# aidanmrli/rwm-pt-pytorch

Measured on AMD Instinct MI355X. Metric: chain-MH-steps/sec, higher is better.
Workload: dtype f32; 1 GPU; BASELINE configs[2]: PT-RWM HIP, RoughCarpet dim=30 modes[-15,0,15], Normal proposal 2.38^2/dim, 32 geometric temps 1->0.01, swap_every=10, 65536 ladders per GPU; dim=30, temps=32, ladders_per_gpu=65536, mh_steps_per_launch=2000, swap_every=10, swap_mode=exchange, swap_order=sequential, rng=Philox4x32-10 in-kernel, world_size=1

## Files before the change

### rwm-pt-pytorch_amd/csrc/kernel.h

```cpp
#pragma once
#include "philox.h"
#include "proposals.h"
#include "targets.h"

namespace ptrwm {

#ifndef PTRWM_BLOCK_THREADS
#define PTRWM_BLOCK_THREADS 256
#endif
constexpr int kBlockThreads = PTRWM_BLOCK_THREADS;
constexpr int kWavesPerBlock = kBlockThreads / 64;
constexpr int kLdsExtraPerThread = 8;
constexpr int kLdsStreamStatPerThread = 5;
constexpr int kStreamSlabs = 2;
constexpr int lds_floats_per_thread(int dp, bool stream) {
  return (stream ? kStreamSlabs * (dp + kLdsStreamStatPerThread) : dp) + kLdsExtraPerThread;
}
constexpr unsigned step_kernel_lds_bytes(int threads, int dp, bool stream = false) {
  return (unsigned)(threads * lds_floats_per_thread(dp, stream)) * 4u;
}
constexpr unsigned kWideVoteBytes = 16u;

struct FullArgs {
  const float *__restrict__ ext_prop;
  const float *__restrict__ ext_u;
  const float *__restrict__ ext_swap_u;
  float *__restrict__ trace;
  float *__restrict__ trace_logp;
  unsigned char *__restrict__ accept_flags;
  long long trace_chains, trace_row0;
  int trace_temps, n_raw_ext;
  int trace_every;
  int steps_to_trace;
  double *__restrict__ mom_sum;
  double *__restrict__ mom_sum_sq;
  double *__restrict__ mom_sum_logp;
  long long *__restrict__ mom_count;
  long long mom_steps;
  int mom_temps, mom_every;
  int steps_to_mom;
};

typedef const __attribute__((address_space(4))) FullArgs *kargs_full_ptr;

struct KArgs {
  float *__restrict__ state;
  float *__restrict__ logp;
  const float *__restrict__ beta;
  const float *__restrict__ temp_scale;
  long long *__restrict__ n_accept;
  double *__restrict__ sq_jump;
  long long *__restrict__ swap_accept;
  long long *__restrict__ last_swap_ordinal;
  long long n_chains, chain_offset, step0;
  long long first_swap_event;
  int n_steps;
  int burn_left;
  int n_temps, dim, swap_every, swap_mode, swap_order, chains_per_wave;
  int steps_to_swap;
  unsigned k0, k1;
  TParams tp;
  PParams pp;
  FullArgs full;
};

__device__ __forceinline__ float swap_log_prob(float bj, float bk, float lj, float lk) {
  return sub_rn(sub_rn(add_rn(mul_rn(bj, lk), mul_rn(bk, lj)), mul_rn(bj, lj)), mul_rn(bk, lk));
}

__device__ __forceinline__ bool swap_accept_test(float u, float log_prob) {
  const float threshold = (log_prob >= 0.0f) ? 1.0f : hw_exp(log_prob);
  return u < threshold;
}

__device__ __forceinline__ bool mh_accept(float beta_t, float lp_new, float lp, float u_acc) {
  const float ratio = mul_rn(beta_t, sub_rn(lp_new, lp));
  return (ratio > 0.0f) || (u_acc < hw_exp(ratio));
}

__device__ __forceinline__ bool swap_pair_plain(int T, int t, float db, float lp, float us) {
  const bool last = t >= T - 1;
  const float u = last ? 0.5f : us;
  const float d = last ? 1.0f : db;
  const float inside = mul_rn(u, sub_rn(1.0f, u));
  return add_rn(__builtin_fminf(inside, d), mul_rn(lp, 0.0f)) > 0.0f;
}
__device__ __forceinline__ bool ladder_votes_plain(bool mine, int first_lane, int lanes_per_ladder) {
  const unsigned long long against = __builtin_amdgcn_ballot_w64(!mine);
  const unsigned long long ladder = (lanes_per_ladder >= 64 ? ~0ull : ((1ull << lanes_per_ladder) - 1ull)) << first_lane;
  return (against & ladder) == 0ull;
}

template <class Sync>
__device__ __forceinline__ void swap_decide(int T, int t, int base, int slot, int swap_mode, int swap_order, int par,
                                            const float *__restrict__ beta, float beta_t, float us, const float *s_l,
                                            float *s_u, int *landed, float &my_l, int &src, bool &pair_acc, Sync sync,
                                            bool plain) {
  if (swap_order == PTRWM_ORDER_SEQUENTIAL) {
    if (swap_mode == PTRWM_SWAP_EXCHANGE) {
      const bool has_k = t < T - 1;
      const float db = has_k ? sub_rn(beta_t, beta[t + 1]) : 1.0f;
      float car_l = s_l[base];
      int car_i = base;
      if (plain) {
        const float lk = s_l[has_k ? slot + 1 : slot];
        s_u[slot] = fmaf(-hw_ln(us), __builtin_amdgcn_rcpf(db), lk);
        sync();
#pragma unroll 2
        for (int j = 0; j < T - 1; ++j) {
          const int ik = base + j + 1;
          const float lkj = s_l[ik];
          const bool ok = car_l < s_u[base + j];
          landed[base + j] = ok ? ik : car_i;
          car_l = ok ? car_l : lkj;
          car_i = ok ? car_i : ik;
        }
      } else {
#pragma unroll 2
        for (int j = 0; j < T - 1; ++j) {
          const float lk = s_l[base + j + 1];
          const float u = s_u[base + j];
          const float bj = beta[j], bk = beta[j + 1];
          const bool ok = swap_accept_test(u, swap_log_prob(bj, bk, car_l, lk));
          const int ik = base + j + 1;
          landed[base + j] = ok ? ik : car_i;
          car_l = ok ? car_l : lk;
          car_i = ok ? car_i : ik;
        }
      }
      landed[base + T - 1] = car_i;
      src = landed[base + t];
      my_l = s_l[src];
      pair_acc = (t < T - 1) && (src == base + t + 1);
    } else {
      if (t < T - 1) {
        const float lk = s_l[slot + 1];
        const bool ok = swap_accept_test(us, swap_log_prob(beta_t, beta[t + 1], my_l, lk));
        if (ok) {
          my_l = lk;
          src = slot + 1;
        }
        pair_acc = ok;
      }
    }
  } else {
    const bool lower = ((t & 1) == par);
    const int partner_t = lower ? t + 1 : t - 1;
    const bool valid = partner_t >= 0 && partner_t < T;
    if (valid) {
      const int partner = base + partner_t;
      const float l_other = s_l[partner];
      const float u_low = lower ? us : s_u[partner];
      const int tj = lower ? t : partner_t;
      const float lj = lower ? my_l : l_other;
      const float lk = lower ? l_other : my_l;
      const bool ok = swap_accept_test(u_low, swap_log_prob(beta[tj], beta[tj + 1], lj, lk));
      if (ok && (lower || swap_mode == PTRWM_SWAP_EXCHANGE)) {
        my_l = l_other;
        src = partner;
      }
      pair_acc = ok && lower;
    }
  }
}

__device__ __forceinline__ int stage_head(const float *g) { return (int)((reinterpret_cast<uintptr_t>(g) >> 2) & 3u); }

template <bool LOAD>
__device__ __forceinline__ void stage_copy(float *__restrict__ lds, float *__restrict__ g, int total, int tid, int nthr) {
  typedef float vec4 __attribute__((ext_vector_type(4)));
  const int head = stage_head(g);
  vec4 *__restrict__ gv = reinterpret_cast<vec4 *>(g - head);
  vec4 *__restrict__ lv = reinterpret_cast<vec4 *>(lds);
  const int v_lo = head ? 1 : 0;
  const int v_hi = (head + total) >> 2;
  constexpr int kDepth = 4;
  int v0 = v_lo + tid;
  for (; v0 + (kDepth - 1) * nthr < v_hi; v0 += kDepth * nthr) {
    vec4 t[kDepth];
#pragma unroll
    for (int k = 0; k < kDepth; ++k) t[k] = LOAD ? gv[v0 + k * nthr] : lv[v0 + k * nthr];
#pragma unroll
    for (int k = 0; k < kDepth; ++k) (LOAD ? lv : gv)[v0 + k * nthr] = t[k];
  }
  if (v0 < v_hi) {
    vec4 t[kDepth - 1];
#pragma unroll
    for (int k = 0; k < kDepth - 1; ++k) {
      const int v = v0 + k * nthr;
      if (v < v_hi) t[k] = LOAD ? gv[v] : lv[v];
    }
#pragma unroll
    for (int k = 0; k < kDepth - 1; ++k) {
      const int v = v0 + k * nthr;
      if (v < v_hi) (LOAD ? lv : gv)[v] = t[k];
    }
  }
  const int e_lo = (4 * v_lo - head < total) ? 4 * v_lo - head : total;
  const int e_hi = (4 * v_hi - head > e_lo) ? 4 * v_hi - head : e_lo;
  if (tid < 6) {
    const int i = tid < 3 ? tid : e_hi + (tid - 3);
    const bool mine = tid < 3 ? (i < e_lo) : (i < total);
    if (mine) {
      if (LOAD) lds[head + i] = g[i];
      else g[i] = lds[head + i];
    }
  }
}

__device__ __forceinline__ int wave_in_block() { return __builtin_amdgcn_readfirstlane((int)(threadIdx.x >> 6)); }
__device__ __forceinline__ int thread_index_now(int wave) {
  unsigned all = ~0u;
  PTRWM_VALUE_BARRIER("+s"(all));
  return wave * 64 + (int)__builtin_amdgcn_mbcnt_hi(all, __builtin_amdgcn_mbcnt_lo(all, 0u));
}

__device__ __forceinline__ void count_add(long long *p, long long v) {
  (void)__hip_atomic_fetch_add(p, v, __ATOMIC_RELAXED, __HIP_MEMORY_SCOPE_AGENT);
}

constexpr unsigned moments_region_doubles(int temps, int dim) { return (unsigned)(temps * (2 * dim + 1)); }

__device__ __forceinline__ void moments_zero(double *reg, int n, int tid, int nthr) {
  for (int i = tid; i < n; i += nthr) reg[i] = 0.0;
}
__device__ __forceinline__ void moments_add(double *p, double v) {
  (void)__hip_atomic_fetch_add(p, v, __ATOMIC_RELAXED, __HIP_MEMORY_SCOPE_WORKGROUP);
}
__device__ __forceinline__ void moments_flush(const double *reg, kargs_full_ptr f, int dim, long long live_ladders, int tid,
                                              int nthr) {
  const int temps = f->mom_temps;
  const int td = temps * dim;
  double *const sum = f->mom_sum, *const sum_sq = f->mom_sum_sq, *const sum_logp = f->mom_sum_logp;
  const int n = 2 * td + (sum_logp != nullptr ? temps : 0);
  for (int i = tid; i < n; i += nthr) {
    const double v = reg[i];
    if (v != 0.0) unsafeAtomicAdd(i < td ? sum + i : (i < 2 * td ? sum_sq + (i - td) : sum_logp + (i - 2 * td)), v);
  }
  long long *const count = f->mom_count;
  const long long add = live_ladders * f->mom_steps;
  if (count != nullptr)
    for (int i = tid; i < temps; i += nthr) count_add(&count[i], add);
}

template <int DP>
__device__ __forceinline__ double *thread_moments_region(float *s_dyn, bool wide, int gthreads, int wave, int stride) {
  float *const base = s_dyn + (wide ? gthreads * (DP + kLdsExtraPerThread) + (int)(kWideVoteBytes / 4u)
                                    : kBlockThreads * (DP + kLdsExtraPerThread));
  return reinterpret_cast<double *>(base) + (wide ? 0 : wave * stride);
}

template <bool EXACT>
__device__ __forceinline__ int fresh_dim(int d0) {
  if constexpr (!EXACT) PTRWM_VALUE_BARRIER("+s"(d0));
  return d0;
}

typedef const __attribute__((address_space(4))) KArgs *kargs_ptr;
__device__ __forceinline__ kargs_ptr late_args() {
  uintptr_t p = (uintptr_t)__builtin_amdgcn_kernarg_segment_ptr();
  PTRWM_VALUE_BARRIER("+s"(p));
  return (kargs_ptr)p;
}

#ifndef PTRWM_J2_FENCE_MASK
#define PTRWM_J2_FENCE_MASK 7
#endif
#ifndef PTRWM_WAVES_SMALL
#define PTRWM_WAVES_SMALL 4
#endif
#ifndef PTRWM_WAVES_40
#define PTRWM_WAVES_40 3
#endif
#ifndef PTRWM_WAVES_MID
#define PTRWM_WAVES_MID 2
#endif
constexpr int min_waves_per_simd(int dp) {
  return dp <= 30 ? PTRWM_WAVES_SMALL : (dp <= 44 ? PTRWM_WAVES_40 : (dp <= 64 ? PTRWM_WAVES_MID : 1));
}
constexpr bool step_loop_at_register_cap(int dp, bool stream) { return !stream && min_waves_per_simd(dp) >= 4 && dp > 24; }

constexpr int stream_waves_per_simd(int dp) {
  return dp <= 10 ? 4 : (dp <= 20 ? 2 : (dp <= 30 ? 2 : 1));
}

constexpr int stream_register_waves(int dp) { return stream_waves_per_simd(dp) < 2 ? 2 : stream_waves_per_simd(dp); }

template <class Target, class Proposal, int DP, bool EXACT, bool FULL, bool STREAM = false>
__global__ void __launch_bounds__(kBlockThreads, STREAM ? stream_register_waves(DP) : min_waves_per_simd(DP)) ptrwm_step_kernel(const KArgs a) {
  static_assert(!(STREAM && FULL), "the streaming form is a production kernel: no fixture / trace arguments");
  const int T = a.n_temps;
  const int D0 = EXACT ? DP : a.dim;
  const int cpw = a.chains_per_wave;
  const bool wide = !STREAM && T > 64;
  const int wave = wave_in_block();
  const int tid = wide ? (int)threadIdx.x : (int)(threadIdx.x & 63);
  long long group = STREAM ? (long long)blockIdx.x * kWavesPerBlock + wave
                           : (wide ? (long long)blockIdx.x : (long long)blockIdx.x * kWavesPerBlock + (threadIdx.x >> 6));
  [[maybe_unused]] const long long n_groups = STREAM ? a.n_chains / cpw : 0;
  [[maybe_unused]] const long long group_stride = STREAM ? (long long)gridDim.x * kWavesPerBlock : 0;
  if (STREAM ? (group >= n_groups) : (group * cpw >= a.n_chains)) return;
  extern __shared__ __attribute__((aligned(16))) float s_dyn[];
  typedef float pf_vec4 __attribute__((ext_vector_type(4)));
  constexpr int NV = STREAM ? (DP + 3) / 4 : 1;
  constexpr int kWaveFloats = 64 * lds_floats_per_thread(DP, STREAM);
  constexpr int kExtra0 = 64 * kStreamSlabs * DP;
  constexpr int kZone0 = kExtra0 + 64 * kLdsExtraPerThread, kZoneFloats = 64 * kLdsStreamStatPerThread;
  [[maybe_unused]] int cur = 0;
  typedef const __attribute__((address_space(1))) void *dma_src;
  typedef __attribute__((address_space(3))) void *dma_dst;
  [[maybe_unused]] auto prefetch = [&](long long g, int slab) {
    const int tid = thread_index_now(wave) & 63;
    const kargs_ptr ap = late_args();
    const int n_vec = (cpw * T * D0) >> 2;
    const int n_live = cpw * T;
    float *const wbase = s_dyn + wave * kWaveFloats;
    const long long r0 = g * n_live;
    float *const zone = wbase + kZone0 + slab * kZoneFloats;
    __builtin_amdgcn_global_load_lds((dma_src)(ap->logp + r0 + (tid < n_live ? tid : 0)), (dma_dst)(uintptr_t)zone, 4, 0, 0);
    if (ap->sq_jump != nullptr && 2 * tid < n_live)
      __builtin_amdgcn_global_load_lds((dma_src)(ap->sq_jump + r0 + 2 * tid), (dma_dst)(uintptr_t)(zone + 64), 16, 0, 0);
    if (ap->n_accept != nullptr && 2 * tid < n_live)
      __builtin_amdgcn_global_load_lds((dma_src)(ap->n_accept + r0 + 2 * tid), (dma_dst)(uintptr_t)(zone + 192), 16, 0, 0);
    const pf_vec4 *__restrict__ gv = reinterpret_cast<const pf_vec4 *>(ap->state + g * cpw * T * (long long)D0);
    float *const dst = wbase + slab * (64 * DP);
#pragma unroll
    for (int k = 0; k < NV; ++k) {
      const int v = tid + 64 * k;
      if (v < n_vec) __builtin_amdgcn_global_load_lds((dma_src)(gv + v), (dma_dst)(uintptr_t)(dst + 256 * k), 16, 0, 0);
    }
  };
  [[maybe_unused]] float beta_t_s = 0.0f, tscale_s = 0.0f;
  [[maybe_unused]] float db_s = 1.0f;
  [[maybe_unused]] pf_vec4 pend_o[NV];
  [[maybe_unused]] float pend_lp = 0.0f;
  [[maybe_unused]] unsigned pend_n_swap = 0u;
  [[maybe_unused]] long long pend_acc = 0;
  [[maybe_unused]] bool pend_acc_on = false;
  [[maybe_unused]] double pend_sq = 0.0;
  [[maybe_unused]] long long pend_ord = 0, pend_group = 0;
  [[maybe_unused]] bool pend_sq_on = false, pend_ord_on = false, have_pending = false;
  [[maybe_unused]] auto flush_pending = [&]() {
    const kargs_ptr ap = late_args();
    const int tid = thread_index_now(wave) & 63;
    const int n_live = cpw * T;
    const int n_vec = (n_live * D0) >> 2;
    pf_vec4 *__restrict__ gv = reinterpret_cast<pf_vec4 *>(ap->state + pend_group * n_live * (long long)D0);
#pragma unroll
    for (int k = 0; k < NV; ++k) {
      const int v = tid + 64 * k;
      if (v < n_vec) gv[v] = pend_o[k];
    }
    if (tid < n_live) {
      const long long r = pend_group * n_live + tid;
      ap->logp[r] = pend_lp;
      if (pend_acc_on) ap->n_accept[r] = pend_acc;
      if (pend_sq_on) ap->sq_jump[r] = pend_sq;
      if (ap->swap_accept != nullptr && pend_n_swap != 0u) count_add(&ap->swap_accept[r], (long long)pend_n_swap);
      if (pend_ord_on) (void)__hip_atomic_fetch_max(&ap->last_swap_ordinal[r], pend_ord, __ATOMIC_RELAXED, __HIP_MEMORY_SCOPE_AGENT);
    }
  };
  if constexpr (STREAM) {
    const int cw_s = tid / T;
    const int t_s = cw_s < cpw ? tid - cw_s * T : 0;
    beta_t_s = a.beta[t_s];
    tscale_s = a.temp_scale[t_s];
    db_s = sub_rn(beta_t_s, a.beta[t_s < T - 1 ? t_s + 1 : t_s]);
    prefetch(group, 0);
  }
  do {
  const long long chain0 = group * cpw;
  const int cw_raw = tid / T;
  const int t_raw = tid - cw_raw * T;
  const bool live = (cw_raw < cpw) && (chain0 + cw_raw < a.n_chains);
  const int cw = live ? cw_raw : 0;
  const int t = live ? t_raw : 0;
  const long long chain = chain0 + cw;
  const long long rep = chain0 * T + (live ? tid : 0);

  float *const s_stage = STREAM ? s_dyn + wave * kWaveFloats + cur * (64 * DP)
                                : s_dyn + (wide ? 0 : (int)(threadIdx.x >> 6) * (64 * (DP + kLdsExtraPerThread)));
  [[maybe_unused]] float *const s_extra = s_dyn + wave * kWaveFloats + kExtra0;
  auto sync_group = [&]() {
    if (wide) {
      __syncthreads();
    } else {
      __builtin_amdgcn_fence(__ATOMIC_ACQ_REL, "wavefront");
      __builtin_amdgcn_wave_barrier();
    }
  };

  float x[DP], y[DP];
  {
    const long long live_chains = (a.n_chains - chain0 < cpw) ? (a.n_chains - chain0) : cpw;
    const int stage_total = (int)live_chains * T * D0;
    float *__restrict__ gs = a.state + chain0 * T * (long long)D0;
    const int nthr = wide ? ((T + 63) & ~63) : 64;
    int row_head = 0;
    if constexpr (!STREAM) {
      stage_copy<true>(s_stage, gs, stage_total, tid, nthr);
      row_head = stage_head(gs);
      if (wide) reinterpret_cast<int *>(s_dyn)[nthr * (DP + kLdsExtraPerThread)] = 0;
      if constexpr (FULL) {
        if (a.full.mom_sum != nullptr) {
          const int n_mom = (int)moments_region_doubles(a.full.mom_temps, D0);
          moments_zero(thread_moments_region<DP>(s_dyn, wide, nthr, wave, n_mom), n_mom, tid, nthr);
        }
      }
    }
    if constexpr (STREAM) asm volatile("s_waitcnt vmcnt(0)" ::: "memory");
    sync_group();
    const float *row = s_stage + row_head + (live ? tid : 0) * D0;
#pragma unroll
    for (int d = 0; d < DP; ++d) x[d] = (d < D0) ? row[d] : 0.0f;
  }
  float lp;
  [[maybe_unused]] double sq_old = 0.0;
  [[maybe_unused]] long long acc_old = 0;
  if constexpr (STREAM) {
    {
      const float *zone = s_dyn + wave * kWaveFloats + kZone0 + cur * kZoneFloats;
      lp = zone[tid];
      if (a.sq_jump != nullptr) sq_old = reinterpret_cast<const double *>(zone + 64)[tid < cpw * T ? tid : 0];
      if (a.n_accept != nullptr) acc_old = reinterpret_cast<const long long *>(zone + 192)[tid < cpw * T ? tid : 0];
    }
    if (have_pending) flush_pending();
    if (group + group_stride < n_groups) prefetch(group + group_stride, cur ^ 1);
  } else {
    lp = a.logp[rep];
  }
  const float beta_t = STREAM ? beta_t_s : a.beta[t];
  const float tscale = STREAM ? tscale_s : a.temp_scale[t];
  bool jump_trusted = false;
  if constexpr (Proposal::kKnowsJump) {
    float xmax = 0.0f;
#pragma unroll
    for (int d = 0; d < DP; ++d) xmax = __builtin_fmaxf(xmax, __builtin_fabsf(x[d]));
    jump_trusted = xmax <= kJumpTrust * Proposal::increment_scale(tscale, a.pp);
  }

  const unsigned long long gchain = (unsigned long long)(a.chain_offset + chain);
  RngCtx rc;
  rc.c2 = (uint32_t)gchain;
  rc.k0 = a.k0;
  rc.k1 = a.k1;
  const uint32_t c3_base = (uint32_t)t | ((uint32_t)(gchain >> 32) << 12);

  unsigned n_acc = 0;
  {
    const int gt = wide ? ((T + 63) & ~63) : 64;
    int *const park = reinterpret_cast<int *>(STREAM ? s_extra + 3 * gt : s_stage + gt * (DP + 3)) + tid;
    park[0] = (int)c3_base;
    park[gt] = 0;
    park[2 * gt] = -1;
    reinterpret_cast<double *>(park - tid + 3 * gt)[tid] = 0.0;
  }
#ifdef PTRWM_NO_SQ_LDS
  double sq_reg = 0.0;
#endif

  const bool ext = FULL && a.full.ext_prop != nullptr;
  const bool trace_on =
      FULL && live && a.full.trace != nullptr && (chain < a.full.trace_chains) && (t < a.full.trace_temps);
  int to_swap = a.steps_to_swap;
  int to_trace = FULL ? a.full.steps_to_trace : 0;
  [[maybe_unused]] int to_mom = FULL ? a.full.steps_to_mom : 0;
  int trace_rows = 0;
  int swap_in_call = 0;
  const int ev_par0 = (int)(a.first_swap_event & 1);
  unsigned long long s = (unsigned long long)a.step0;

  for (int i = 0; i < a.n_steps; ++i, ++s) {
    const bool count_on = i >= a.burn_left;
    --to_swap;
    const bool multiple = (to_swap == 0);
    if (multiple) to_swap = a.swap_every;
    const bool swap_due = multiple && count_on && (T > 1);

    rc.c0hi = (uint32_t)(s >> 32) << 16;
    rc.c1 = (uint32_t)s;
    rc.c3 = c3_base | (kStreamMH << 8);
#ifndef PTRWM_NO_C2_OPAQUE
    if constexpr (step_loop_at_register_cap(DP, STREAM)) asm volatile("" : "+v"(rc.c2));
#endif

    long long srep = 0;
    const float *ext_raw = nullptr;
    float ext_u = 0.0f;
    if constexpr (FULL) {
      srep = ((long long)i * a.n_chains + chain) * T + t;
      if (ext) {
        ext_raw = a.full.ext_prop + srep * a.full.n_raw_ext;
        ext_u = a.full.ext_u[srep];
      }
    }

    constexpr int W = canon_width(DP);
    float jump = 0.0f;
    int jump_kind;
    const float u_acc = Proposal::propose(y, x, fresh_dim<EXACT>(D0), tscale, a.pp, rc, ext_raw, ext_u, jump, jump_kind);
    const float lp_new = Target::template logp<false>(y, fresh_dim<EXACT>(D0), a.tp);
    const int D = fresh_dim<EXACT>(D0);

    const bool acc = mh_accept(beta_t, lp_new, lp, u_acc);
    const float lp_mh = acc ? lp_new : lp;
    if constexpr (FULL) {
      if (a.full.accept_flags != nullptr && live) a.full.accept_flags[srep] = acc ? 1 : 0;
    }

    float j2;
    if (!swap_due && jump_kind != kJumpNone) {
      float from_states = 0.0f;
      if (!jump_trusted) {
        PTRWM_COLD_PATH();
        float j2p[4] = {0.0f, 0.0f, 0.0f, 0.0f};
        PTRWM_DIM_LOOP(d, DP, D, {
          const float dl = sub_rn(y[d], x[d]);
          j2p[d / W] = fmaf(dl, dl, j2p[d / W]);
        })
        from_states = tree4_add(j2p);
      }
      PTRWM_DIM_LOOP(d, DP, D, {
        x[d] = acc ? y[d] : x[d];
        if ((d & PTRWM_J2_FENCE_MASK) == PTRWM_J2_FENCE_MASK) sched_fence_soft();
      })
      j2 = acc ? (jump_trusted ? jump : from_states) : 0.0f;
      lp = lp_mh;
    } else if (!swap_due) {
      float j2p[4] = {0.0f, 0.0f, 0.0f, 0.0f};
#ifdef PTRWM_J2_SEPARATE
#pragma unroll
      for (int d = 0; d < DP; ++d) {
        if (d < D) {
          const float dl = sub_rn(y[d], x[d]);
          j2p[d / W] = fmaf(dl, dl, j2p[d / W]);
        }
        if ((d & PTRWM_J2_FENCE_MASK) == PTRWM_J2_FENCE_MASK) sched_fence_soft();
      }
#pragma unroll
      for (int d = 0; d < DP; ++d)
        if (d < D) x[d] = acc ? y[d] : x[d];
#else
      PTRWM_DIM_LOOP(d, DP, D, {
        const float dl = sub_rn(y[d], x[d]);
        j2p[d / W] = fmaf(dl, dl, j2p[d / W]);
        x[d] = acc ? y[d] : x[d];
        if ((d & PTRWM_J2_FENCE_MASK) == PTRWM_J2_FENCE_MASK) sched_fence_soft();
      })
#endif
      j2 = tree4_add(j2p);
      if (!acc) j2 = 0.0f;
      lp = lp_mh;
    } else {
      const int tid_s = thread_index_now(wave);
      const int slot = wide ? tid_s : (tid_s & 63);
      const int group_threads = wide ? ((T + 63) & ~63) : 64;
      float *const rows = STREAM ? s_dyn + wave * kWaveFloats + cur * (64 * DP)
                                 : s_dyn + (wide ? 0 : (tid_s >> 6) * (64 * (DP + kLdsExtraPerThread)));
      float *const s_l = STREAM ? s_dyn + wave * kWaveFloats + kExtra0 : rows + group_threads * DP;
      float *const s_u = s_l + group_threads;
      int *const park = reinterpret_cast<int *>(s_l + 3 * group_threads) + slot;
      const uint32_t c3_s = (uint32_t)park[0];
      const int t = (int)(c3_s & 0xffu);
      const int base = live ? slot - t : 0;
      int src = slot;
      float my_l = lp_mh;
      bool pair_acc = false;
      float us;
      if (ext) {
        us = (t < T - 1) ? a.full.ext_swap_u[((long long)swap_in_call * a.n_chains + chain) * (T - 1) + t] : 2.0f;
      } else {
        const u32x4 r = philox4x32_10(rc.c0hi, rc.c1, rc.c2, c3_s | (kStreamSwap << 8), rc.k0, rc.k1);
        us = u01(r.x);
      }
      s_l[slot] = my_l;
      s_u[slot] = us;
      const bool pair_plain = swap_pair_plain(T, t, STREAM ? db_s : sub_rn(beta_t, a.beta[t < T - 1 ? t + 1 : t]), my_l, us);
      bool swap_plain;
      if (wide) {
        int *const objection = reinterpret_cast<int *>(s_l + kLdsExtraPerThread * group_threads);
        if (!pair_plain) *objection = swap_in_call + 1;
        sync_group();
        swap_plain = *objection != swap_in_call + 1;
      } else {
        swap_plain = ladder_votes_plain(pair_plain, base, T);
        sync_group();
      }
      swap_decide(T, t, base, slot, a.swap_mode, a.swap_order, (ev_par0 + swap_in_call) & 1, a.beta, beta_t, us, s_l, s_u,
                  reinterpret_cast<int *>(s_u + group_threads), my_l, src, pair_acc, sync_group, swap_plain);
      if (pair_acc) {
        park[group_threads] += 1;
        park[2 * group_threads] = swap_in_call;
      }
      {
        float j2p[4] = {0.0f, 0.0f, 0.0f, 0.0f};
        float *my_row = rows + slot * D;
        PTRWM_DIM_LOOP(d, DP, D, { my_row[d] = acc ? y[d] : x[d]; })
        sync_group();
        const int Dr = fresh_dim<EXACT>(D0);
        const float *src_row = rows + src * Dr;
        PTRWM_DIM_LOOP(d, DP, Dr, {
          const float w = src_row[d];
          const float dl = sub_rn(w, x[d]);
          j2p[d / W] = fmaf(dl, dl, j2p[d / W]);
          x[d] = w;
          if ((d & 7) == 7) sched_fence_soft();
        })
        j2 = tree4_add(j2p);
      }
      lp = my_l;
      ++swap_in_call;
    }

    if (count_on) {
      n_acc += acc ? 1u : 0u;
#ifdef PTRWM_NO_SQ_LDS
      sq_reg += (double)j2;
#else
      const int tid_q = thread_index_now(wave);
      const int gt_q = wide ? ((T + 63) & ~63) : 64;
      double *const sq_slot = reinterpret_cast<double *>(
                                  STREAM ? s_dyn + wave * kWaveFloats + kExtra0 + 6 * 64
                                         : s_dyn + (wide ? 0 : wave * (64 * (DP + kLdsExtraPerThread))) + gt_q * (DP + 6)) +
                              (wide ? tid_q : (tid_q & 63));
      (void)__hip_atomic_fetch_add(sq_slot, (double)j2, __ATOMIC_RELAXED, __HIP_MEMORY_SCOPE_WAVEFRONT);
#endif
    }
    if constexpr (FULL) {
      bool trace_now = false;
      if (a.full.trace != nullptr) {
        --to_trace;
        trace_now = (to_trace == 0);
        if (trace_now) to_trace = a.full.trace_every;
      }
      if (trace_now && trace_on) {
        const long long row = ((a.full.trace_row0 + trace_rows) * a.full.trace_chains + chain) * a.full.trace_temps + t;
        float *__restrict__ tr = a.full.trace + row * D;
        PTRWM_DIM_LOOP(d, DP, D, { tr[d] = x[d]; })
        if (a.full.trace_logp != nullptr) a.full.trace_logp[row] = lp;
      }
      trace_rows += trace_now ? 1 : 0;
      if (a.full.mom_sum != nullptr) {
        --to_mom;
        const bool mom_now = (to_mom == 0);
        if (mom_now) to_mom = a.full.mom_every;
        if (mom_now && count_on && live && t < a.full.mom_temps) {
          const int mt = a.full.mom_temps;
          double *const reg = thread_moments_region<DP>(s_dyn, wide, wide ? ((T + 63) & ~63) : 64, wave,
                                                        (int)moments_region_doubles(mt, D));
          double *const rs = reg + t * D;
          double *const rq = reg + (mt + t) * D;
          PTRWM_DIM_LOOP(d, DP, D, {
            const double v = (double)x[d];
            moments_add(rs + d, v);
            moments_add(rq + d, v * v);
          })
          moments_add(reg + 2 * mt * D + t, (double)lp);
        }
      }
    }
  }

  const kargs_ptr ae = late_args();
  long long c0_out;
  {
    const int T2 = fresh_dim<false>(T), D2 = EXACT ? DP : fresh_dim<false>(D0), cpw2 = fresh_dim<false>(cpw);
    const bool wide2 = T2 > 64;
    const int tx2 = thread_index_now(wave);
    const int tid2 = wide2 ? tx2 : (tx2 & 63);
    float *const rows2 = STREAM ? s_dyn + wave * kWaveFloats + cur * (64 * DP)
                                : s_dyn + (wide2 ? 0 : wave * (64 * (DP + kLdsExtraPerThread)));
    long long c0;
    if constexpr (STREAM) {
      c0 = group * cpw2;
    } else {
      const long long bid = (long long)fresh_dim<false>((int)blockIdx.x);
      c0 = (wide2 ? bid : bid * kWavesPerBlock + wave) * cpw2;
    }
    const long long n_chains2 = ae->n_chains;
    const long long live_chains = (n_chains2 - c0 < cpw2) ? (n_chains2 - c0) : cpw2;
    const int stage_total = (int)live_chains * T2 * D2;
    const long long stage_g0 = c0 * T2 * (long long)D2;
    c0_out = c0;
    float *__restrict__ gs = ae->state + stage_g0;
    sync_group();
    if (live) {
      float *row = rows2 + stage_head(gs) + tid2 * D2;
#pragma unroll
      for (int d = 0; d < DP; ++d)
        if (d < D2) row[d] = x[d];
    }
    sync_group();
    const int nthr = wide2 ? ((T2 + 63) & ~63) : 64;
    if constexpr (FULL) {
      const kargs_full_ptr fa = &ae->full;
      if (fa->mom_sum != nullptr)
        moments_flush(thread_moments_region<DP>(s_dyn, wide2, nthr, wave, (int)moments_region_doubles(fa->mom_temps, D2)),
                      fa, D2, live_chains, tid2, nthr);
    }
    if constexpr (STREAM) {
      const pf_vec4 *__restrict__ lv = reinterpret_cast<const pf_vec4 *>(rows2);
      const int n_vec = stage_total >> 2;
#pragma unroll
      for (int k = 0; k < NV; ++k) {
        const int v = tid2 + 64 * k;
        if (v < n_vec) pend_o[k] = lv[v];
      }
    } else {
      stage_copy<false>(rows2, gs, stage_total, tid2, nthr);
    }
  }
  if (live) {
    const int tid_o = thread_index_now(wave);
    const int T_o = fresh_dim<false>(T);
    const long long rep = c0_out * T_o + (T_o > 64 ? tid_o : (tid_o & 63));
    const int gt_o = T_o > 64 ? ((T_o + 63) & ~63) : 64;
    const int *const park = reinterpret_cast<const int *>(STREAM ? s_dyn + wave * kWaveFloats + kExtra0 + 3 * 64
                                                                 : s_dyn + (T_o > 64 ? 0 : (tid_o >> 6) * (64 * (DP + kLdsExtraPerThread)))
                                                                       + gt_o * (DP + 3)) + (T_o > 64 ? tid_o : (tid_o & 63));
    const int t = park[0] & 0xff;
    const unsigned n_swap_acc = (unsigned)park[gt_o];
    const int last_event = park[2 * gt_o];
    const int tid_g = T_o > 64 ? tid_o : (tid_o & 63);
#ifdef PTRWM_NO_SQ_LDS
    const double sq = sq_reg;
#else
    const double sq = reinterpret_cast<const double *>(park - tid_g + 3 * gt_o)[tid_g];
#endif
    if constexpr (STREAM) {
      pend_lp = lp;
      pend_acc_on = ae->n_accept != nullptr && n_acc != 0u;
      pend_acc = acc_old + (long long)n_acc;
      pend_n_swap = n_swap_acc;
      pend_sq_on = ae->sq_jump != nullptr && sq != 0.0;
      pend_sq = sq_old + sq;
      pend_ord_on = ae->last_swap_ordinal != nullptr && last_event >= 0;
      const long long ev = ae->first_swap_event + last_event;
      pend_ord = (ae->swap_order == PTRWM_ORDER_SEQUENTIAL) ? ev * (T_o - 1) + t + 1 : ev + 1;
    } else {
    ae->logp[rep] = lp;
    if (ae->n_accept != nullptr && n_acc != 0u) count_add(&ae->n_accept[rep], (long long)n_acc);
    if (ae->sq_jump != nullptr && sq != 0.0) ae->sq_jump[rep] += sq;
    if (ae->swap_accept != nullptr && n_swap_acc != 0u) count_add(&ae->swap_accept[rep], (long long)n_swap_acc);
    if (ae->last_swap_ordinal != nullptr && last_event >= 0) {
      const long long ev = ae->first_swap_event + last_event;
      const long long ord = (ae->swap_order == PTRWM_ORDER_SEQUENTIAL) ? ev * (T_o - 1) + t + 1 : ev + 1;
      if (ord > ae->last_swap_ordinal[rep]) ae->last_swap_ordinal[rep] = ord;
    }
    }
  }
  if constexpr (!STREAM) break;
  pend_group = group;
  have_pending = true;
  group += group_stride;
  cur ^= 1;
  } while (group < n_groups);
  if constexpr (STREAM) flush_pending();
}

template <class Target, int DP>
__global__ void __launch_bounds__(kBlockThreads) ptrwm_logdensity_kernel(const float *__restrict__ x,
                                                                          float *__restrict__ out,
                                                                          long long n, int D, TParams tp) {
  const long long i = (long long)blockIdx.x * kBlockThreads + threadIdx.x;
  if (i >= n) return;
  float y[DP];
  const float *__restrict__ xp = x + i * D;
#pragma unroll
  for (int d = 0; d < DP; ++d) y[d] = (d < D) ? xp[d] : 0.0f;
  out[i] = Target::template logp<true>(y, D, tp);
}

constexpr int standalone_min_waves(int dp) { return dp > 64 ? 2 : 1; }

template <class Proposal, int DP>
__global__ void __launch_bounds__(kBlockThreads, standalone_min_waves(DP)) ptrwm_propose_kernel(
    float *__restrict__ out, long long n, int D, int T, const float *__restrict__ temp_scale, PParams pp,
    const float *__restrict__ ext_raw, int n_raw_ext, unsigned k0, unsigned k1) {
  const long long i = (long long)blockIdx.x * kBlockThreads + threadIdx.x;
  if (i >= n * T) return;
  const long long row = i / T;
  const int t = (int)(i - row * T);
  float x[DP], y[DP];
#pragma unroll
  for (int d = 0; d < DP; ++d) x[d] = 0.0f;
  RngCtx rc;
  rc.c0hi = (uint32_t)((unsigned long long)row >> 32) << 16;
  rc.c1 = (uint32_t)row;
  rc.c2 = 0;
  rc.c3 = (uint32_t)t | (kStreamMH << 8);
  rc.k0 = k0;
  rc.k1 = k1;
  const float *er = ext_raw != nullptr ? ext_raw + i * n_raw_ext : nullptr;
  float jump = 0.0f;
  int jump_kind;
  Proposal::propose(y, x, D, temp_scale[t], pp, rc, er, 0.0f, jump, jump_kind);
  float *__restrict__ op = out + i * D;
#pragma unroll
  for (int d = 0; d < DP; ++d)
    if (d < D) op[d] = y[d];
}

constexpr unsigned split_tile_lds_bytes(int dim) { return (unsigned)(64 * dim + 4) * 4u; }

template <class Proposal, int DP>
__global__ void __launch_bounds__(64, standalone_min_waves(DP)) ptrwm_split_propose_kernel(
    const float *__restrict__ state, float *__restrict__ proposals, float *__restrict__ accept_u, long long n_chains,
    long long chain_offset, unsigned long long step, int D, int T, const float *__restrict__ temp_scale, PParams pp,
    const float *__restrict__ ext_raw, const float *__restrict__ ext_u, int n_raw_ext, unsigned k0, unsigned k1,
    const long long *__restrict__ device_step) {
  extern __shared__ __attribute__((aligned(16))) float s_tile[];
  const int lane = (int)threadIdx.x;
  const long long n_reps = n_chains * T;
  const long long first = (long long)blockIdx.x * 64;
  if (first >= n_reps) return;
  if (device_step != nullptr) step += (unsigned long long)*device_step;
  const int n_rows = (n_reps - first < 64) ? (int)(n_reps - first) : 64;
  const bool live = lane < n_rows;
  const long long i = first + (live ? lane : 0);
  const long long chain = i / T;
  const int t = (int)(i - chain * T);
  float x[DP], y[DP];
  float *__restrict__ gx = const_cast<float *>(state) + first * D;
  stage_copy<true>(s_tile, gx, n_rows * D, lane, 64);
  __builtin_amdgcn_fence(__ATOMIC_ACQ_REL, "wavefront");
  __builtin_amdgcn_wave_barrier();
  {
    const float *row = s_tile + stage_head(gx) + (live ? lane : 0) * D;
#pragma unroll
    for (int d = 0; d < DP; ++d) x[d] = (d < D) ? row[d] : 0.0f;
  }
  const unsigned long long gchain = (unsigned long long)(chain_offset + chain);
  RngCtx rc;
  rc.c0hi = (uint32_t)(step >> 32) << 16;
  rc.c1 = (uint32_t)step;
  rc.c2 = (uint32_t)gchain;
  rc.c3 = (uint32_t)t | ((uint32_t)(gchain >> 32) << 12) | (kStreamMH << 8);
  rc.k0 = k0;
  rc.k1 = k1;
  const float *er = ext_raw != nullptr ? ext_raw + i * n_raw_ext : nullptr;
  float jump = 0.0f;
  int jump_kind;
  const float u = Proposal::propose(y, x, D, temp_scale[t], pp, rc, er, ext_u != nullptr ? ext_u[i] : 0.0f, jump, jump_kind);
  float *__restrict__ gy = proposals + first * D;
  __builtin_amdgcn_fence(__ATOMIC_ACQ_REL, "wavefront");
  __builtin_amdgcn_wave_barrier();
  if (live) {
    float *row = s_tile + stage_head(gy) + lane * D;
#pragma unroll
    for (int d = 0; d < DP; ++d)
      if (d < D) row[d] = y[d];
  }
  __builtin_amdgcn_fence(__ATOMIC_ACQ_REL, "wavefront");
  __builtin_amdgcn_wave_barrier();
  stage_copy<false>(s_tile, gy, n_rows * D, lane, 64);
  if (!live) return;
  accept_u[i] = u;
  float xmax = 0.0f;
#pragma unroll
  for (int d = 0; d < DP; ++d) xmax = __builtin_fmaxf(xmax, __builtin_fabsf(x[d]));
  const bool trusted = Proposal::kKnowsJump && xmax <= kJumpTrust * Proposal::increment_scale(temp_scale[t], pp);
  accept_u[n_reps + i] = (jump_kind == kJumpTotal && trusted) ? jump : -1.0f;
}

}
```

Measured before the change: 46.59 billion chain-MH-steps/s.

## Split MH step loop into swap-free inner runs ending in a swap step

Restructures the per-step loop so an inner loop runs plain MH steps until the next swap boundary. The swap path is taken only at the tail step of each run, which removes the per-step swap_due check and the three-way branch from the hot path. The commit and statistics logic moves into always-inline lambdas that are reused in both places. In exchange, code size grows because the commit path is duplicated, and the count_on/burn-in handling at run boundaries becomes more intricate.

```diff
diff --git a/rwm-pt-pytorch_amd/csrc/kernel.h b/rwm-pt-pytorch_amd/csrc/kernel.h
--- a/rwm-pt-pytorch_amd/csrc/kernel.h
+++ b/rwm-pt-pytorch_amd/csrc/kernel.h
@@ -470,46 +470,10 @@
   const int ev_par0 = (int)(a.first_swap_event & 1);
   unsigned long long s = (unsigned long long)a.step0;
 
-  for (int i = 0; i < a.n_steps; ++i, ++s) {
-    const bool count_on = i >= a.burn_left;
-    --to_swap;
-    const bool multiple = (to_swap == 0);
-    if (multiple) to_swap = a.swap_every;
-    const bool swap_due = multiple && count_on && (T > 1);
-
-    rc.c0hi = (uint32_t)(s >> 32) << 16;
-    rc.c1 = (uint32_t)s;
-    rc.c3 = c3_base | (kStreamMH << 8);
-#ifndef PTRWM_NO_C2_OPAQUE
-    if constexpr (step_loop_at_register_cap(DP, STREAM)) asm volatile("" : "+v"(rc.c2));
-#endif
-
-    long long srep = 0;
-    const float *ext_raw = nullptr;
-    float ext_u = 0.0f;
-    if constexpr (FULL) {
-      srep = ((long long)i * a.n_chains + chain) * T + t;
-      if (ext) {
-        ext_raw = a.full.ext_prop + srep * a.full.n_raw_ext;
-        ext_u = a.full.ext_u[srep];
-      }
-    }
-
-    constexpr int W = canon_width(DP);
-    float jump = 0.0f;
-    int jump_kind;
-    const float u_acc = Proposal::propose(y, x, fresh_dim<EXACT>(D0), tscale, a.pp, rc, ext_raw, ext_u, jump, jump_kind);
-    const float lp_new = Target::template logp<false>(y, fresh_dim<EXACT>(D0), a.tp);
-    const int D = fresh_dim<EXACT>(D0);
-
-    const bool acc = mh_accept(beta_t, lp_new, lp, u_acc);
-    const float lp_mh = acc ? lp_new : lp;
-    if constexpr (FULL) {
-      if (a.full.accept_flags != nullptr && live) a.full.accept_flags[srep] = acc ? 1 : 0;
-    }
-
+  constexpr int W = canon_width(DP);
+  auto commit_plain = [&](bool acc, float jump, int jump_kind, int D) __attribute__((always_inline)) -> float {
     float j2;
-    if (!swap_due && jump_kind != kJumpNone) {
+    if (jump_kind != kJumpNone) {
       float from_states = 0.0f;
       if (!jump_trusted) {
         PTRWM_COLD_PATH();
@@ -525,8 +489,7 @@
         if ((d & PTRWM_J2_FENCE_MASK) == PTRWM_J2_FENCE_MASK) sched_fence_soft();
       })
       j2 = acc ? (jump_trusted ? jump : from_states) : 0.0f;
-      lp = lp_mh;
-    } else if (!swap_due) {
+    } else {
       float j2p[4] = {0.0f, 0.0f, 0.0f, 0.0f};
 #ifdef PTRWM_J2_SEPARATE
 #pragma unroll
@@ -550,6 +513,111 @@
 #endif
       j2 = tree4_add(j2p);
       if (!acc) j2 = 0.0f;
+    }
+    return j2;
+  };
+  auto finish_step = [&](bool count_on, bool acc, float j2, int D) __attribute__((always_inline)) {
+    if (count_on) {
+      n_acc += acc ? 1u : 0u;
+#ifdef PTRWM_NO_SQ_LDS
+      sq_reg += (double)j2;
+#else
+      const int tid_q = thread_index_now(wave);
+      const int gt_q = wide ? ((T + 63) & ~63) : 64;
+      double *const sq_slot = reinterpret_cast<double *>(
+                                  STREAM ? s_dyn + wave * kWaveFloats + kExtra0 + 6 * 64
+                                         : s_dyn + (wide ? 0 : wave * (64 * (DP + kLdsExtraPerThread))) + gt_q * (DP + 6)) +
+                              (wide ? tid_q : (tid_q & 63));
+      (void)__hip_atomic_fetch_add(sq_slot, (double)j2, __ATOMIC_RELAXED, __HIP_MEMORY_SCOPE_WAVEFRONT);
+#endif
+    }
+    if constexpr (FULL) {
+      bool trace_now = false;
+      if (a.full.trace != nullptr) {
+        --to_trace;
+        trace_now = (to_trace == 0);
+        if (trace_now) to_trace = a.full.trace_every;
+      }
+      if (trace_now && trace_on) {
+        const long long row = ((a.full.trace_row0 + trace_rows) * a.full.trace_chains + chain) * a.full.trace_temps + t;
+        float *__restrict__ tr = a.full.trace + row * D;
+        PTRWM_DIM_LOOP(d, DP, D, { tr[d] = x[d]; })
+        if (a.full.trace_logp != nullptr) a.full.trace_logp[row] = lp;
+      }
+      trace_rows += trace_now ? 1 : 0;
+      if (a.full.mom_sum != nullptr) {
+        --to_mom;
+        const bool mom_now = (to_mom == 0);
+        if (mom_now) to_mom = a.full.mom_every;
+        if (mom_now && count_on && live && t < a.full.mom_temps) {
+          const int mt = a.full.mom_temps;
+          double *const reg = thread_moments_region<DP>(s_dyn, wide, wide ? ((T + 63) & ~63) : 64, wave,
+                                                        (int)moments_region_doubles(mt, D));
+          double *const rs = reg + t * D;
+          double *const rq = reg + (mt + t) * D;
+          PTRWM_DIM_LOOP(d, DP, D, {
+            const double v = (double)x[d];
+            moments_add(rs + d, v);
+            moments_add(rq + d, v * v);
+          })
+          moments_add(reg + 2 * mt * D + t, (double)lp);
+        }
+      }
+    }
+  };
+
+  int i = 0;
+  while (i < a.n_steps) {
+    const int left = a.n_steps - i;
+    const bool to_multiple = to_swap <= left;
+    int run = to_multiple ? to_swap : left;
+    to_swap = to_multiple ? a.swap_every : to_swap - left;
+    bool count_on, acc;
+    float lp_mh;
+    float jump;
+    int jump_kind;
+    int D;
+    for (;; ++i, ++s) {
+      count_on = i >= a.burn_left;
+      rc.c0hi = (uint32_t)(s >> 32) << 16;
+      rc.c1 = (uint32_t)s;
+      rc.c3 = c3_base | (kStreamMH << 8);
+#ifndef PTRWM_NO_C2_OPAQUE
+      if constexpr (step_loop_at_register_cap(DP, STREAM)) asm volatile("" : "+v"(rc.c2));
+#endif
+
+      long long srep = 0;
+      const float *ext_raw = nullptr;
+      float ext_u = 0.0f;
+      if constexpr (FULL) {
+        srep = ((long long)i * a.n_chains + chain) * T + t;
+        if (ext) {
+          ext_raw = a.full.ext_prop + srep * a.full.n_raw_ext;
+          ext_u = a.full.ext_u[srep];
+        }
+      }
+
+      jump = 0.0f;
+      const float u_acc = Proposal::propose(y, x, fresh_dim<EXACT>(D0), tscale, a.pp, rc, ext_raw, ext_u, jump, jump_kind);
+      const float lp_new = Target::template logp<false>(y, fresh_dim<EXACT>(D0), a.tp);
+      D = fresh_dim<EXACT>(D0);
+
+      acc = mh_accept(beta_t, lp_new, lp, u_acc);
+      lp_mh = acc ? lp_new : lp;
+      if constexpr (FULL) {
+        if (a.full.accept_flags != nullptr && live) a.full.accept_flags[srep] = acc ? 1 : 0;
+      }
+
+      if (--run == 0) break;
+      const float j2 = commit_plain(acc, jump, jump_kind, D);
+      lp = lp_mh;
+      finish_step(count_on, acc, j2, D);
+    }
+    const bool swap_due = to_multiple && count_on && (T > 1);
+
+    float j2;
+    if (!swap_due) {
+      j2 = commit_plain(acc, jump, jump_kind, D);
       lp = lp_mh;
     } else {
       const int tid_s = thread_index_now(wave);
@@ -611,54 +679,9 @@
       lp = my_l;
       ++swap_in_call;
     }
-
-    if (count_on) {
-      n_acc += acc ? 1u : 0u;
-#ifdef PTRWM_NO_SQ_LDS
-      sq_reg += (double)j2;
-#else
-      const int tid_q = thread_index_now(wave);
-      const int gt_q = wide ? ((T + 63) & ~63) : 64;
-      double *const sq_slot = reinterpret_cast<double *>(
-                                  STREAM ? s_dyn + wave * kWaveFloats + kExtra0 + 6 * 64
-                                         : s_dyn + (wide ? 0 : wave * (64 * (DP + kLdsExtraPerThread))) + gt_q * (DP + 6)) +
-                              (wide ? tid_q : (tid_q & 63));
-      (void)__hip_atomic_fetch_add(sq_slot, (double)j2, __ATOMIC_RELAXED, __HIP_MEMORY_SCOPE_WAVEFRONT);
-#endif
-    }
-    if constexpr (FULL) {
-      bool trace_now = false;
-      if (a.full.trace != nullptr) {
-        --to_trace;
-        trace_now = (to_trace == 0);
-        if (trace_now) to_trace = a.full.trace_every;
-      }
-      if (trace_now && trace_on) {
-        const long long row = ((a.full.trace_row0 + trace_rows) * a.full.trace_chains + chain) * a.full.trace_temps + t;
-        float *__restrict__ tr = a.full.trace + row * D;
-        PTRWM_DIM_LOOP(d, DP, D, { tr[d] = x[d]; })
-        if (a.full.trace_logp != nullptr) a.full.trace_logp[row] = lp;
-      }
-      trace_rows += trace_now ? 1 : 0;
-      if (a.full.mom_sum != nullptr) {
-        --to_mom;
-        const bool mom_now = (to_mom == 0);
-        if (mom_now) to_mom = a.full.mom_every;
-        if (mom_now && count_on && live && t < a.full.mom_temps) {
-          const int mt = a.full.mom_temps;
-          double *const reg = thread_moments_region<DP>(s_dyn, wide, wide ? ((T + 63) & ~63) : 64, wave,
-                                                        (int)moments_region_doubles(mt, D));
-          double *const rs = reg + t * D;
-          double *const rq = reg + (mt + t) * D;
-          PTRWM_DIM_LOOP(d, DP, D, {
-            const double v = (double)x[d];
-            moments_add(rs + d, v);
-            moments_add(rq + d, v * v);
-          })
-          moments_add(reg + 2 * mt * D + t, (double)lp);
-        }
-      }
-    }
+    finish_step(count_on, acc, j2, D);
+    ++i;
+    ++s;
   }
 
   const kargs_ptr ae = late_args();
```

After: 47.24 billion chain-MH-steps/s, median of 6. 1.4% higher.
